# tho-kn/EgoTAP

Measured on AMD Instinct MI355X. Metric: stereo frames/sec (2D->3D lift, B=256, 256x256), higher is better.
Workload: dtype f32; 1 GPU; UnrealEgo 16-joint lifting head (heatmaps [B,90,64,64] -> joints [B,16,3]), forward only, fp32, batch 256 per GPU, inputs resident in HBM; batch_per_gpu=256, global_batch=256, heatmap=64, parallelism=dp1 (batch shards, no collective)

## Files before the change

### egotap_amd/csrc/egotap_abi.hip

```cpp
#include <stdarg.h>
#include <stdio.h>
#include <string.h>

#include <string>
#include <unordered_map>
#include <vector>

#include "attention_f32.h"
#include "common.h"
#include "conv_f32.h"
#include "conv_bf16.h"
#include "gemm_f32.h"
#include "gemm_bf16.h"
#include "gemm_bf16_dma.h"
#include "gemm_f32_dma.h"
#include "attention_bf16.h"
#include "layernorm.h"
#include "metrics.h"
#include "heatmap_synth.h"
#include "pu_chain.h"
#include "gemm_tn_bf16.h"
#include "train_ops.h"
#include "gemm_bf16s.h"
#include "gemm_bf16s64.h"
// ... 86 lines not shown

struct HmParams {
    struct Bn { const float *g, *b, *m, *v; long long* nbt; };
    const float* stem_w; Bn stem_bn;
    struct Block { const float *w1, *w2, *wd; Bn bn1, bn2, bnd; } blk[4][6];
    int nblk[4];
    struct Cv { const float *w, *b; } l1x1[4], up[3], head;
    int n_out;
};

struct egotap_handle_s {
    egotap_config cfg;
    int J, T, grid, ppd, side, seq, C, D, H, hid, out_joints;
    std::unordered_map<std::string, int64_t> expect[EGOTAP_NET_COUNT];
    std::unordered_map<std::string, Param> bound[EGOTAP_NET_COUNT];
    bool lift_resolved = false;
    LiftParams lp;
    std::unordered_map<std::string, Param> bound_grad;
    bool grad_resolved = false;
    LiftParams lg;
    bool hm_resolved[EGOTAP_NET_COUNT] = {false, false, false};
    HmParams hp[EGOTAP_NET_COUNT];
    int debug_stop = 0;
    int pu_resident[2] = {-1, -1};
    bool pu_chain = true;
    unsigned* pu_fault_host = nullptr;
    unsigned* pu_fault_dev = nullptr;
    int pu_faults = 0;
    int pu_debug_drop = 0;
    int precision = EGOTAP_PREC_F32;
    __bf16* wscratch = nullptr;
    size_t wscratch_bytes = 0;
    __bf16* ascratch = nullptr;
    size_t ascratch_bytes = 0;
    __bf16* conv_pack = nullptr;
    float* conv_part = nullptr;
    size_t conv_part_floats = 0;
    bool timing = false;
    std::vector<hipEvent_t> ev;
    struct Rec { const char* role; const char* kernel; double flops; };
    std::vector<Rec> rec;
    size_t ev_used = 0;
    std::string detail;
};
typedef egotap_handle_s Handle;

// ... 276 lines not shown
        : h(h_), s(s_), on(h_ && h_->timing) {
        if (!on) return;
        if (h->ev_used + 2 > h->ev.size()) {
            hipEvent_t a, b;
            if (hipEventCreate(&a) != hipSuccess || hipEventCreate(&b) != hipSuccess) { on = false; return; }
            h->ev.push_back(a);
            h->ev.push_back(b);
        }
        (void)hipEventRecord(h->ev[h->ev_used], s);
        h->rec.push_back({role, kernel, flops});
    }
    ~GemmTimer() {
        if (!on) return;
        (void)hipEventRecord(h->ev[h->ev_used + 1], s);
        h->ev_used += 2;
    }
};

template <class AL> struct AlName;
template <> struct AlName<ALoadPlain> { static constexpr const char* v = "ALoadPlain"; };
template <> struct AlName<ALoadPatch> { static constexpr const char* v = "ALoadPatch"; };
template <> struct AlName<ALoadTokens> { static constexpr const char* v = "ALoadTokens"; };
template <> struct AlName<ALoadLive> { static constexpr const char* v = "ALoadLive"; };
template <> struct AlName<ALoadRot> { static constexpr const char* v = "ALoadRot"; };
template <> struct AlName<ALoadStereo> { static constexpr const char* v = "ALoadStereo"; };
template <> struct AlName<ALoadStereoGated> { static constexpr const char* v = "ALoadStereoGated"; };
template <class E> struct EpiName;
template <> struct EpiName<EpiBias> { static constexpr const char* v = "EpiBias"; };
template <> struct EpiName<EpiBiasRes> { static constexpr const char* v = "EpiBiasRes"; };
template <> struct EpiName<EpiBiasResLive> { static constexpr const char* v = "EpiBiasResLive"; };
template <> struct EpiName<EpiBiasGelu> { static constexpr const char* v = "EpiBiasGelu"; };
template <> struct EpiName<EpiBnLrelu> { static constexpr const char* v = "EpiBnLrelu"; };
template <> struct EpiName<EpiPatch> { static constexpr const char* v = "EpiPatch"; };

template <class Cfg, class AL, class Epi>
static hipError_t gemm(Handle* h, const char* role, const AL& al, const SegMat& W, const Epi& epi, float* C, long ldc,
                       int M, int N, int K, hipStream_t s) {
    static const std::string kname = std::string("gemm_f32_kernel<") + std::to_string(Cfg::BM) + "x" +
                                     std::to_string(Cfg::BN) + "x" + std::to_string(Cfg::BK) + "," + AlName<AL>::v + "," +
                                     EpiName<Epi>::v + ">";
    GemmTimer t(h, s, role, kname.c_str(), 2.0 * M * N * K);
    return gemm_f32_launch<Cfg, AL, Epi>(al, W, epi, C, ldc, M, N, K, s);
}

static int device_cu_count() {
    static int n = 0;
    if (n == 0) {
        int dev = 0, v = 0;
        if (hipGetDevice(&dev) == hipSuccess && hipDeviceGetAttribute(&v, hipDeviceAttributeMultiprocessorCount, dev) == hipSuccess && v > 0) n = v;
        else n = 256;
    }
    return n;
}
// ... 36 lines not shown
        hipError_t e = hipGetLastError();
        if (e != hipSuccess) return e;
        if constexpr (std::is_same<AL, ALoadPlain>::value) {
            if (K % DmaCfg::BK == 0 && N % DmaCfg::BN == 0 && W.seg % DmaCfg::BN == 0 && al.lda % 4 == 0 && M >= 1024) {
                __bf16* a = (size_t)M * K * 2 <= h->ascratch_bytes ? h->ascratch : nullptr;
                if (a) {
                    const long a8 = (long)M * K / 8;
                    hipLaunchKernelGGL(f32_to_bf16_rows_kernel, dim3((unsigned)((a8 + 255) / 256)), dim3(256), 0, s, al.A, al.lda, a, K / 8, a8);
                    e = hipGetLastError();
                    if (e != hipSuccess) return e;
                    return gemm_bf16_dma_launch(a, (long)K, B, epi, C, ldc, M, N, K, device_cu_count(), s);
                }
            }
        }
        return gemm_bf16_persist_launch<BfCfg<1, 1>, AL, Epi, SegMatB>(al, B, epi, C, ldc, M, N, K, device_cu_count(), s);
    }
    return gemm_bf16_persist_launch<BfCfg<1, 1>, AL, Epi>(al, W, epi, C, ldc, M, N, K, device_cu_count(), s);
}

template <class AL, class Epi>
static hipError_t gemm_big(Handle* h, const char* role, const AL& al, const SegMat& W, const Epi& epi, float* C, long ldc,
                           int M, int N, int K, hipStream_t s) {
    using Cfg = PipeD;
    if (h && h->precision == EGOTAP_PREC_BF16X3) {
        static const std::string kname3 = std::string("gemm_bf16_persist_kernel<256x256x16,bf16x3,") + AlName<AL>::v + "," + EpiName<Epi>::v + ">";
        GemmTimer t(h, s, role, kname3.c_str(), 2.0 * M * N * K);
        return gemm_bf16_persist_launch<BfCfg<3, 1>, AL, Epi>(al, W, epi, C, ldc, M, N, K, device_cu_count(), s);
    }
    if (h && h->precision == EGOTAP_PREC_BF16) {
        static const std::string kname1 = std::string("gemm_bf16_persist_kernel<256x256x32,bf16,") + AlName<AL>::v + "," + EpiName<Epi>::v + ">";
        GemmTimer t(h, s, role, kname1.c_str(), 2.0 * M * N * K);
        return gemm_bf16_plain(h, al, W, epi, C, ldc, M, N, K, s);
    }
    if constexpr (AL::HAS_PTR) {
        if (N % DmaF32Cfg::BN == 0 && K % DmaF32Cfg::BK == 0 && W.seg % DmaF32Cfg::BN == 0 && W.ld % 4 == 0 && al.dma_ok()) {
            static const std::string kdma = std::string("gemm_f32_dma_kernel<256x256x16,") + AlName<AL>::v + "," + EpiName<Epi>::v + ">";
            GemmTimer t(h, s, role, kdma.c_str(), 2.0 * M * N * K);
            return gemm_f32_dma_launch(al, W, epi, C, ldc, M, N, K, device_cu_count(), s);
        }
    }
    static const std::string kname = std::string("gemm_f32_persist_kernel<256x256x16,") + AlName<AL>::v + "," + EpiName<Epi>::v + ">";
    GemmTimer t(h, s, role, kname.c_str(), 2.0 * M * N * K);
    return gemm_f32_persist_launch<Cfg, AL, Epi>(al, W, epi, C, ldc, M, N, K, device_cu_count(), s);
}

static constexpr size_t SPLITK_FLOATS = (size_t)1 << 24;
enum { GS_BIG = 0, GS_DIRECT_A, GS_DIRECT_S, GS_SPLIT_S, GS_SPLIT_A, GS_HYBRID };
struct SmallRoute { int kind, splits, head_rows; };
template <class E> struct epi_row_free : std::false_type {};
template <> struct epi_row_free<EpiBias> : std::true_type {};
template <> struct epi_row_free<EpiBiasGelu> : std::true_type {};
template <> struct epi_row_free<EpiBnLrelu> : std::true_type {};
template <> struct epi_row_free<EpiNone> : std::true_type {};
static SmallRoute gemm_small_route(const Handle* h, bool plain_loader, int M, int N, int K, int wseg, int cus, bool row_free = false) {
    const long tiles256 = (long)((M + 255) / 256) * ((N + 255) / 256);
    const long fill = (h && h->precision != EGOTAP_PREC_F32) ? 64 : 160;
    if (N % 128 != 0 || K % 32 != 0 || wseg % 128 != 0) return SmallRoute{GS_BIG, 1, 0};
    if (tiles256 >= fill) {
        if (plain_loader && h && h->precision == EGOTAP_PREC_F32 && tiles256 < 4L * cus) {
            const double t_round = K * 0.2319 + 5.0;
            const double t_big = (double)((tiles256 + cus - 1) / cus) * t_round;
            const double t_direct = gemm_f32_direct_estimate_us<TileA>(M, N, K, cus);
            if (row_free && N % 256 == 0 && tiles256 > cus) {
                const int tn = N / 256, mh = (int)((tiles256 / cus) * cus / tn);
                const int Mt = M - mh * 256;
                if (mh >= 1 && Mt > 0) {
// ... 102 lines not shown
    w.HPB = w.HPA + al256((size_t)B * H * 4);
    w.FAULT = take(64);
    w.SPLITK = take(SPLITK_FLOATS);
    w.total = o;
    return w;
}

#if EGOTAP_IN(0)
extern "C" int egotap_lift_workspace_bytes(egotap_handle h, int B, size_t* bytes) {
    EGO_CHECK(h && bytes, "null argument");
    EGO_CHECK(B >= 0, "negative batch");
    *bytes = lift_ws(h, B > 0 ? B : 1).total;
    return EGOTAP_OK;
}
#endif

#if EGOTAP_IN(0)
extern "C" int egotap_lift_intermediate(egotap_handle h, int B, const char* name, size_t* offset, int64_t* numel) {
    EGO_CHECK(h && name && offset && numel, "null argument");
    const LiftWs w = lift_ws(h, B > 0 ? B : 1);
    const int64_t M = (int64_t)B * h->seq;
    if (!strcmp(name, "tokens")) { *offset = w.Y; *numel = M * h->D; }
    else if (!strcmp(name, "x")) { *offset = w.X; *numel = M * h->D; }
    else if (!strcmp(name, "pos_embed")) { *offset = w.POSZ; *numel = (int64_t)B * h->T * h->hid; }
    else if (!strcmp(name, "rot_embed")) { *offset = w.ROTZ; *numel = (int64_t)B * h->T * h->hid; }
    else if (!strcmp(name, "skel_embed")) { *offset = w.HS1; *numel = (int64_t)h->J * B * h->H; }
    else { egotap_set_error("unknown intermediate '%s'", name); return EGOTAP_ERR_INVALID; }
    return EGOTAP_OK;
}
#endif

#if EGOTAP_IN(0)
extern "C" int egotap_set_pu_chain(egotap_handle h, int enable) {
    EGO_CHECK(h, "null handle");
    h->pu_chain = enable != 0;
    h->pu_resident[0] = h->pu_resident[1] = -1;
    return EGOTAP_OK;
}
extern "C" int egotap_debug_pu_drop_workgroups(egotap_handle h, int n) {
    EGO_CHECK(h && n >= 0 && n < 16, "egotap_debug_pu_drop_workgroups: n in [0, 16)");
    h->pu_debug_drop = n;
    return EGOTAP_OK;
}
extern "C" int egotap_pu_chain_status(egotap_handle h, int* enabled, int* faults) {
    EGO_CHECK(h, "null handle");
    if (h->pu_fault_host && __atomic_load_n(h->pu_fault_host, __ATOMIC_RELAXED) != 0u) {
// ... 18 lines not shown
extern "C" int egotap_set_weight_scratch(egotap_handle h, void* buf, size_t bytes) {
    EGO_CHECK(h, "null handle");
    EGO_CHECK(((uintptr_t)buf & 15) == 0, "egotap_set_weight_scratch: 16-byte alignment");
    h->wscratch = (__bf16*)buf;
    h->wscratch_bytes = buf ? bytes : 0;
    return EGOTAP_OK;
}
#endif

#if EGOTAP_IN(0)
extern "C" int egotap_set_act_scratch(egotap_handle h, void* buf, size_t bytes) {
    EGO_CHECK(h, "null handle");
    EGO_CHECK(((uintptr_t)buf & 15) == 0, "egotap_set_act_scratch: 16-byte alignment");
    h->ascratch = (__bf16*)buf;
    h->ascratch_bytes = buf ? bytes : 0;
    return EGOTAP_OK;
}
#endif

#if EGOTAP_IN(0)
extern "C" int egotap_lift_debug_stop(egotap_handle h, int stage) {
    EGO_CHECK(h, "null handle");
    h->debug_stop = stage;
    return EGOTAP_OK;
}
#endif

template <class Epi>
static hipError_t fc1_nt(Handle* h, int which, const __bf16* src, const __bf16* w, long K, const Epi& ep, int BT, int cus, hipStream_t s) {
    const int HW = h->cfg.hm_size * h->cfg.hm_size;
    const bool deep = g_gemm_bf16s_bk != 32 && K % 64 == 0 && K >= 128 && (which == 0 ? h->D % 64 == 0 : HW % 64 == 0) && (long)256 * K * 2 < (1L << 31);
    if (which == 0) {
        const size_t tok_bytes = (size_t)(BT / h->T) * h->seq * h->D * 2;
        if (deep && g_conv_addressing == 0 && tok_bytes < ((size_t)1 << 32) - 4096)
            return gemm_bf16s64_launch_x(X64TokensS{src, 0u, h->T, h->D, h->seq, h->side, h->ppd, h->grid}, w, K, ep, BT, 2048, (int)K, cus, s);
        if (deep) return gemm_bf16s64_launch_x(X64Tokens{src, h->T, h->D, h->seq, h->side, h->ppd, h->grid}, w, K, ep, BT, 2048, (int)K, cus, s);
        return gemm_bf16s_launch(XTokens{src, h->T, h->D, h->seq, h->side, h->ppd, h->grid}, w, K, ep, BT, 2048, (int)K, cus, s);
    }
    const size_t hm_bytes = (size_t)(BT / (2 * h->J)) * h->C * HW * 2;
    if (deep && g_conv_addressing == 0 && hm_bytes < ((size_t)1 << 32) - 4096) return gemm_bf16s64_launch_x(X64RotS{src, 0u, h->C, h->J, HW}, w, K, ep, BT, 2048, (int)K, cus, s);
    if (deep) return gemm_bf16s64_launch_x(X64Rot{src, h->C, h->J, HW}, w, K, ep, BT, 2048, (int)K, cus, s);
    return gemm_bf16s_launch(XRot{src, h->C, h->J, HW}, w, K, ep, BT, 2048, (int)K, cus, s);
}

static hipError_t launch_ln(const float* x, float* y, const float* g, const float* b, int rows, float eps, hipStream_t s) {
    if (rows <= 0) return hipSuccess;
// ... 9 lines not shown
        const SmallRoute r = gemm_small_route(h, true, M, D, K, D, device_cu_count());
        if ((r.kind == GS_SPLIT_S || r.kind == GS_SPLIT_A) && r.splits > 1) {
            static const std::string kname = "gemm_f32_splitk_kernel<ALoadPlain>+splitk_reduce_res_ln_kernel";
            GemmTimer t(h, s, role, kname.c_str(), 2.0 * M * D * K);
            hipError_t e = r.kind == GS_SPLIT_S ? gemm_f32_splitk_partials<TileS>(ALoadPlain{A, lda}, segmat1(Wp, D, K), P, SPLITK_FLOATS, M, D, K, s, r.splits)
                                                : gemm_f32_splitk_partials<TileA>(ALoadPlain{A, lda}, segmat1(Wp, D, K), P, SPLITK_FLOATS, M, D, K, s, r.splits);
            if (e != hipSuccess) return e;
            hipLaunchKernelGGL(splitk_reduce_res_ln_kernel<1024>, dim3(min((M + 3) / 4, 256 * 8)), dim3(256), 0, s, (const float*)P, bias, (const float*)X, X, ln_g,
                               ln_b, Y, M, r.splits, 1e-12f);
            return hipGetLastError();
        }
    }
    hipError_t e = gemm_small(h, role, ALoadPlain{A, lda}, segmat1(Wp, D, K), EpiBiasRes{segvec1(bias, D), X, D}, X, D, M, D, K, P, s);
    if (e != hipSuccess) return e;
    return launch_ln(X, Y, ln_g, ln_b, M, 1e-12f, s);
}

static ALoadPlain rebase(const ALoadPlain& a, int m0) { return ALoadPlain{a.A + (long)m0 * a.lda, a.lda}; }
static ALoadLive rebase(ALoadLive a, int m0) { a.lr.m0 += m0; return a; }
static EpiBias rebase(const EpiBias& e, int) { return e; }
static EpiBiasGelu rebase(const EpiBiasGelu& e, int) { return e; }
static EpiBiasRes rebase(EpiBiasRes e, int m0) { e.R += (long)m0 * e.ldr; return e; }
static EpiBiasResLive rebase(EpiBiasResLive e, int m0) { e.lr.m0 += m0; return e; }
template <class AL, class Epi>
static hipError_t gemm_rounds(Handle* h, const char* role, const AL& al, const SegMat& W, const Epi& epi, float* C, long ldc, int M, int N, int K,
                              hipStream_t s) {
    const int cus = device_cu_count(), tn = N / 256;
    const long tiles = (long)((M + 255) / 256) * tn;
    const int mh = (int)((tiles / cus) * cus / tn) * 256;
    if (N % 256 == 0 && K % 32 == 0 && mh > 0 && mh < M) {
        const double t_round = K * 0.2319 + 5.0;
        const double t_big = (double)((tiles + cus - 1) / cus) * t_round;
        const double t_split = (double)(((long)(mh / 256) * tn + cus - 1) / cus) * t_round + 4.0 + gemm_f32_direct_estimate_us<TileA>(M - mh, N, K, cus);
        if (t_split < t_big) {
            hipError_t e = gemm_big(h, role, al, W, epi, C, ldc, mh, N, K, s);
            if (e != hipSuccess) return e;
            return gemm<TileA>(h, role, rebase(al, mh), W, rebase(epi, mh), C + (long)mh * ldc, ldc, M - mh, N, K, s);
        }
    }
    return gemm_big(h, role, al, W, epi, C, ldc, M, N, K, s);
}

static bool lift_prune_last(Handle* h, int B) {
#ifdef EGOTAP_ATTN_F32_LIVE
    const int D = h->D, M = B * h->seq, Nq = h->T * h->ppd * h->ppd;
    if (h->precision != EGOTAP_PREC_F32 || h->debug_stop != 0 || h->cfg.vit_layers < 1 || Nq < 32 || Nq >= h->seq || D % 256 != 0) return false;
    const int cus = device_cu_count();
    if (gemm_small_route(h, true, M, 3 * D, D, D, cus, true).kind != GS_BIG || gemm_small_route(h, true, M, D, D, D, cus).kind != GS_BIG ||
        gemm_small_route(h, true, M, 4 * D, D, 4 * D, cus, true).kind != GS_BIG || gemm_small_route(h, true, M, D, 4 * D, D, cus).kind != GS_BIG)
        return false;
    return attention_f32_ksplit(B, h->seq, h->cfg.vit_heads, SPLITK_FLOATS, cus) == 1;
#else
    (void)h; (void)B;
    return false;
#endif
}

static int lift_forward_impl(Handle* h, const float* hm, int B, float* pose, void* ws, size_t ws_bytes, void* stream, bool pose_only,
                             const char* who) {
    EGO_CHECK(h, "null handle");
    if (B == 0) return EGOTAP_OK;
    EGO_CHECK(B > 0 && hm && pose && ws, "%s: null argument or negative batch", who);
    EGO_CHECK(((uintptr_t)hm & 15) == 0 && ((uintptr_t)ws & 255) == 0, "hm must be 16-byte and ws 256-byte aligned");
    int rc = lift_resolve(h);
    if (rc != EGOTAP_OK) return rc;
    const LiftWs w = lift_ws(h, B);
    if (ws_bytes < w.total) {
        egotap_set_error("workspace too small: %zu bytes given, %zu needed for B=%d", ws_bytes, w.total, B);
        return EGOTAP_ERR_WORKSPACE;
    }
    hipStream_t s = (hipStream_t)stream;
    const LiftParams& p = h->lp;
    char* base = (char*)ws;
    auto F = [&](size_t off) { return (float*)(base + off); };
    float *X = F(w.X), *Y = F(w.Y), *QKV = F(w.QKV), *CTX = F(w.CTX), *HID = F(w.HID);
    float* SPK = F(w.SPLITK);
    float *Z1 = F(w.Z1), *Z2 = F(w.Z2), *POSZ = F(w.POSZ), *ROTZ = F(w.ROTZ);
    float *F0 = F(w.F0), *G0 = F(w.G0), *HS0 = F(w.HS0), *F1 = F(w.F1), *G1 = F(w.G1), *HS1 = F(w.HS1);
// ... 63 lines not shown
            const XTokens xt{Yb, h->T, D, h->seq, h->side, h->ppd, h->grid};
            const int sp = gemm_bf16s_ksplit(BT, 2048, K1, cu, SPLITK_FLOATS);
            if (sp > 1) EGO_HIP(gemm_bf16s_splitk_launch(xt, Wb, (long)K1, bnf(p.pos_fc[0], Z1), SPK, sp, BT, 2048, K1, cu, s));
            else EGO_HIP(fc1_nt(h, 0, Yb, Wb, (long)K1, bnf(p.pos_fc[0], Z1), BT, cu, s));
            EGO_HIP((fc_gemm(h, "pos_fc2", ALoadPlain{Z1, 2048}, segmat1(p.pos_fc[1].w, 512, 2048), bn(p.pos_fc[1]), Z2, 512, BT, 512, 2048, SPK, s)));
            EGO_HIP((fc_gemm(h, "pos_fc3", ALoadPlain{Z2, 512}, segmat1(p.pos_fc[2].w, hid, 512), bn(p.pos_fc[2]), POSZ, hid, BT, hid, 512, SPK, s)));
        }
        {
            __bf16* hmb = HIDb;
            const long n8 = (long)B * h->C * HW / 8;
            hipLaunchKernelGGL(f32_to_bf16_kernel, dim3((unsigned)((n8 + 255) / 256)), dim3(256), 0, s, hm, hmb, n8);
            prep(p.rot_fc[0].w, Wb, 2048, 2 * HW);
            EGO_HIP(hipGetLastError());
            const XRot xr{hmb, h->C, J, HW};
            const int sp = gemm_bf16s_ksplit(BT, 2048, 2 * HW, cu, SPLITK_FLOATS);
            if (sp > 1) EGO_HIP(gemm_bf16s_splitk_launch(xr, Wb, 2L * HW, bnf(p.rot_fc[0], Z1), SPK, sp, BT, 2048, 2 * HW, cu, s));
            else EGO_HIP(fc1_nt(h, 1, hmb, Wb, 2L * HW, bnf(p.rot_fc[0], Z1), BT, cu, s));
            EGO_HIP((fc_gemm(h, "rot_fc2", ALoadPlain{Z1, 2048}, segmat1(p.rot_fc[1].w, 512, 2048), bn(p.rot_fc[1]), Z2, 512, BT, 512, 2048, SPK, s)));
            EGO_HIP((fc_gemm(h, "rot_fc3", ALoadPlain{Z2, 512}, segmat1(p.rot_fc[2].w, hid, 512), bn(p.rot_fc[2]), ROTZ, hid, BT, hid, 512, SPK, s)));
        }
    } else {
    const int NL = h->cfg.vit_layers;
    const bool prune = pose_only && lift_prune_last(h, B);
    EGO_HIP(launch_ln(X, Y, NL > 0 ? p.layer[0].ln1_g : p.lnf_g, NL > 0 ? p.layer[0].ln1_b : p.lnf_b, M, 1e-12f, s));
    for (int i = 0; i < NL; ++i) {
        const auto& L = p.layer[i];
#ifdef EGOTAP_ATTN_F32_LIVE
        if (prune && i + 1 == NL) {
            const LiveRows lr{h->seq, h->side, h->ppd, h->grid, h->T};
            const int Nq = h->T * h->ppd * h->ppd, Mc = B * Nq;
            float* Xc = QKV;
            SegMat Wkv; Wkv.p[0] = L.k_w; Wkv.p[1] = L.v_w; Wkv.p[2] = L.v_w; Wkv.seg = D; Wkv.ld = D;
            SegVec bkv; bkv.p[0] = L.k_b; bkv.p[1] = L.v_b; bkv.p[2] = L.v_b; bkv.seg = D;
            EGO_HIP((gemm_big(h, "kv", ALoadPlain{Y, D}, Wkv, EpiBias{bkv}, QKV + D, 3L * D, M, 2 * D, D, s)));
            EGO_HIP((gemm_rounds(h, "q_live", ALoadLive{Y, D, lr}, segmat1(L.q_w, D, D), EpiBias{segvec1(L.q_b, D)}, QKV, 3L * D, Mc, D, D, s)));
            EGO_HIP(attention_f32_live_launch(QKV, 3L * D, Nq, QKV, CTX, B, h->seq, h->cfg.vit_heads, s));
            EGO_HIP((gemm_rounds(h, "attn_out_live", ALoadPlain{CTX, D}, segmat1(L.o_w, D, D), EpiBiasResLive{segvec1(L.o_b, D), X, D, lr}, Xc, D, Mc, D, D, s)));
            EGO_HIP(launch_ln(Xc, Y, L.ln2_g, L.ln2_b, Mc, 1e-12f, s));
            EGO_HIP((gemm_rounds(h, "mlp_up_live", ALoadPlain{Y, D}, segmat1(L.up_w, 4 * D, D), EpiBiasGelu{segvec1(L.up_b, 4 * D)}, HID, 4L * D, Mc, 4 * D, D, s)));
            EGO_HIP((gemm_rounds(h, "mlp_down_live", ALoadPlain{HID, 4L * D}, segmat1(L.dn_w, D, 4 * D), EpiBiasRes{segvec1(L.dn_b, D), Xc, D}, Xc, D, Mc, D, 4 * D, s)));
            EGO_HIP(launch_ln(Xc, Y, p.lnf_g, p.lnf_b, Mc, 1e-12f, s));
            break;
        }
#endif
        {
            SegMat Wqkv; Wqkv.p[0] = L.q_w; Wqkv.p[1] = L.k_w; Wqkv.p[2] = L.v_w; Wqkv.seg = D; Wqkv.ld = D;
            SegVec bqkv; bqkv.p[0] = L.q_b; bqkv.p[1] = L.k_b; bqkv.p[2] = L.v_b; bqkv.seg = D;
            EGO_HIP((gemm_small(h, "qkv", ALoadPlain{Y, D}, Wqkv, EpiBias{bqkv}, QKV, 3L * D, M, 3 * D, D, SPK, s)));
        }
        if (h->precision == EGOTAP_PREC_BF16X3 && h->seq % 32 == 0) EGO_HIP(attention_bf16_launch<3>(QKV, CTX, B, h->seq, h->cfg.vit_heads, s));
        else if (h->precision == EGOTAP_PREC_BF16 && h->seq % 32 == 0) EGO_HIP(attention_bf16_launch<1>(QKV, CTX, B, h->seq, h->cfg.vit_heads, s));
        else EGO_HIP(attention_f32_launch(QKV, CTX, B, h->seq, h->cfg.vit_heads, s, nullptr, SPK, SPLITK_FLOATS, device_cu_count()));
        EGO_HIP(gemm_res_ln(h, "attn_out", CTX, D, L.o_w, L.o_b, X, M, D, D, L.ln2_g, L.ln2_b, Y, SPK, s));
        EGO_HIP((gemm_small(h, "mlp_up", ALoadPlain{Y, D}, segmat1(L.up_w, 4 * D, D), EpiBiasGelu{segvec1(L.up_b, 4 * D)}, HID, 4L * D, M, 4 * D, D, SPK, s)));
        const bool last = i + 1 == NL;
        EGO_HIP(gemm_res_ln(h, "mlp_down", HID, 4L * D, L.dn_w, L.dn_b, X, M, D, 4 * D, last ? p.lnf_g : p.layer[i + 1].ln1_g, last ? p.lnf_b : p.layer[i + 1].ln1_b, Y,
                            SPK, s));
        if (h->debug_stop == 2 + i) return EGOTAP_OK;
    }
    auto bn = [](const LiftParams::Fc& f) { return EpiBnLrelu{f.b, f.g, f.beta, f.mean, f.var, 1e-5f, 0.2f}; };
    const bool skinny_fc1 = BT < SKINNY_ROWS || (h->precision == EGOTAP_PREC_F32 && (long)((BT + 255) / 256) * (2048 / 256) < 100);
    {
        const int K1 = h->ppd * h->ppd * D;
        auto fc1 = [&](const auto& al) -> hipError_t {
            if (skinny_fc1 && BT <= 64)
                return gemm_f32_splitk_launch<TileS>(al, segmat1(p.pos_fc[0].w, 2048, K1), bn(p.pos_fc[0]), Z1, 2048, SPK, SPLITK_FLOATS, BT, 2048, K1, s, device_cu_count());
            if (skinny_fc1)
                return gemm_f32_splitk_launch<TileA>(al, segmat1(p.pos_fc[0].w, 2048, K1), bn(p.pos_fc[0]), Z1, 2048, SPK, SPLITK_FLOATS, BT, 2048, K1, s);
            return gemm_big(h, "pos_fc1", al, segmat1(p.pos_fc[0].w, 2048, K1), bn(p.pos_fc[0]), Z1, 2048, BT, 2048, K1, s);
        };
        if (prune) EGO_HIP(fc1(ALoadPlain{Y, (long)K1}));
// ... 2556 lines not shown
```

### egotap_amd/csrc/gemm_f32.h

```cpp
#pragma once
#include "common.h"
#include <type_traits>

struct ALoadPlain {
    const float* A;
    long lda;
    struct Row { const float* p; };
    __device__ __forceinline__ Row row(int m) const { return Row{A + (long)m * lda}; }
    __device__ __forceinline__ f32x4 load(const Row& r, int k) const { return *(const f32x4*)(r.p + k); }
    static constexpr bool HAS_PTR = true;
    __device__ __forceinline__ const float* ptr(const Row& r, int k) const { return r.p + k; }
    __host__ bool dma_ok() const { return lda % 4 == 0 && lda < (1L << 21) && ((uintptr_t)A & 15) == 0; }
};

struct ALoadPatch {
    const float* hm;
    int C, S, seq, side, ppd, grid, T;
    const float* zeros = nullptr;
    struct Row { const float* p; };
    static constexpr bool HAS_PTR = true;
    __device__ __forceinline__ const float* ptr(const Row& r, int k) const { return r.p ? r.p + (k >> 4) * S + (k & 15) : zeros + k; }
    __host__ bool dma_ok() const { return zeros != nullptr && S % 4 == 0 && ((uintptr_t)hm & 15) == 0 && ((uintptr_t)zeros & 15) == 0; }
    __device__ __forceinline__ Row row(int m) const {
        const int b = m / seq, tok = m - b * seq;
// ... 33 lines not shown
struct LiveRows {
    int seq, side, ppd, grid, T;
    int m0 = 0;
    __host__ __device__ __forceinline__ long phys(int m) const {
        m += m0;
        const int pp = ppd * ppd, L = T * pp;
        const int b = m / L, r = m - b * L, i = r / pp, s = r - i * pp;
        const int pr = (i / grid) * ppd + s / ppd, pc = (i % grid) * ppd + s % ppd;
        return (long)b * seq + pr * side + pc;
    }
};
struct ALoadLive {
    const float* A;
    long lda;
    LiveRows lr;
    struct Row { const float* p; };
    __device__ __forceinline__ Row row(int m) const { return Row{A + lr.phys(m) * lda}; }
    __device__ __forceinline__ f32x4 load(const Row& r, int k) const { return *(const f32x4*)(r.p + k); }
    static constexpr bool HAS_PTR = true;
    __device__ __forceinline__ const float* ptr(const Row& r, int k) const { return r.p + k; }
    __host__ bool dma_ok() const { return lda % 4 == 0 && lda < (1L << 21) && ((uintptr_t)A & 15) == 0; }
};

struct ALoadRot {
    const float* hm;
    int C, J, HW;
    struct Row { const float* p; };
    __device__ __forceinline__ Row row(int m) const {
        const int T = 2 * J;
        const int b = m / T, t = m - b * T;
        const int eye = t / J, j = t - eye * J;
        return Row{hm + (long)(b * C + 2 * J + eye * 2 * J + j) * HW};
    }
    __device__ __forceinline__ f32x4 load(const Row& r, int k) const {
        const int cs = k / HW;
        return *(const f32x4*)(r.p + (long)cs * J * HW + (k - cs * HW));
    }
    static constexpr bool HAS_PTR = true;
    __device__ __forceinline__ const float* ptr(const Row& r, int k) const {
        const int cs = k / HW;
        return r.p + (long)cs * J * HW + (k - cs * HW);
    }
    __host__ bool dma_ok() const { return HW % 4 == 0 && ((uintptr_t)hm & 15) == 0; }
};

struct ALoadStereo {
// ... 204 lines not shown
};

struct EpiScatterPatch : EpiNone {
    float* hm;
    int C, S, seq, side, ppd, grid, T;
    __device__ __forceinline__ float* dst(int m, int n) const {
        const int b = m / seq, tok = m - b * seq;
        const int pr = tok / side, pc = tok - pr * side;
        const int cell = (pr / ppd) * grid + pc / ppd;
        if (cell >= T) return nullptr;
        return hm + ((long)(b * C + cell) * S + (pr % ppd) * 16 + (n >> 4)) * S + (pc % ppd) * 16 + (n & 15);
    }
};
struct EpiScatterRot : EpiNone {
    float* hm;
    int C, J, HW;
    __device__ __forceinline__ float* dst(int m, int n) const {
        const int T = 2 * J;
        const int b = m / T, t = m - b * T;
        const int eye = t / J, j = t - eye * J, cs = n / HW;
        return hm + (long)(b * C + 2 * J + eye * 2 * J + cs * J + j) * HW + (n - cs * HW);
    }
};
template <class E> struct epi_scatters : std::false_type {};
template <> struct epi_scatters<EpiScatterPatch> : std::true_type {};
template <> struct epi_scatters<EpiScatterRot> : std::true_type {};
template <class Epi>
__device__ __forceinline__ void epi_store(const Epi& epi, float* C, long ldc, int m, int n, float v) {
    if constexpr (epi_scatters<Epi>::value) {
        if (float* p = epi.dst(m, n)) *p = v;
    } else {
        C[(long)m * ldc + n] = v;
    }
}
template <class Epi>
__device__ __forceinline__ void epi_store4(const Epi& epi, float* C, long ldc, int m, int n0, const f32x4& v) {
    if constexpr (epi_scatters<Epi>::value) {
        if (float* p = epi.dst(m, n0)) *(f32x4*)p = v;
    } else {
        *(f32x4*)(C + (long)m * ldc + n0) = v;
    }
}

template <int BM_, int BN_, int BK_, int WM_, int WN_, int MINW_>
struct GemmCfg {
    static constexpr int BM = BM_, BN = BN_, BK = BK_, WM = WM_, WN = WN_, MINW = MINW_;
    static constexpr int THREADS = 64 * WM * WN;
// ... 648 lines not shown
```

### egotap_amd/csrc/gemm_f32_dma.h

```cpp
#pragma once
#include <type_traits>
#include "gemm_f32.h"
#include "lds_dma.h"

struct DmaF32Cfg {
    static constexpr int BM = 256, BN = 256, BK = 16, WM = 4, WN = 2, THREADS = 512, NS = 4, TM = 2, TN = 4;
    static constexpr int ROWB = 64;
    static constexpr int STAGE = (BM + BN) * ROWB;
    static constexpr int ELD = 36, EPATCH = 16 * ELD * 4;
    static constexpr int LDS_BYTES = NS * STAGE + (THREADS / 64) * EPATCH;
    static_assert(LDS_BYTES <= 160 * 1024, "LDS budget");
};

template <class ALoad, class Epi>
__global__ __launch_bounds__(DmaF32Cfg::THREADS, 2) void gemm_f32_dma_kernel(ALoad al, SegMat W, Epi epi, float* C,
                                                                          long ldc, int M, int N, int K, int tiles_m, int tiles_n) {
    using Cfg = DmaF32Cfg;
    constexpr int BM = Cfg::BM, BN = Cfg::BN, BK = Cfg::BK, NS = Cfg::NS, TM = Cfg::TM, TN = Cfg::TN, ROWB = Cfg::ROWB, ELD = Cfg::ELD;
    extern __shared__ __attribute__((aligned(16))) char smem_dmaf[];
    const int tid = threadIdx.x, lane = tid & 63, wid = tid >> 6;
    const int wm = wid / Cfg::WN, wn = wid % Cfg::WN;
    const int l31 = lane & 31, lh = lane >> 5;
    float* Es = (float*)(smem_dmaf + NS * Cfg::STAGE + wid * Cfg::EPATCH);

// ... 194 lines not shown
            after_epi = true;
            {
                int tm_, tn_;
                tile_of(c_tile, tm_, tn_);
                constexpr bool DUAL = sizeof(typename Epi::Col4) <= 16 && !(Epi::HAS_RES && sizeof(typename Epi::Col4) < 16);
                if (DUAL && (tm_ + 1) * BM <= M) epilogue(std::integral_constant<bool, DUAL>{});
                else epilogue(std::false_type{});
            }
            c_kt = 0;
            ++c_tile;
        }
    }
    asm volatile("s_waitcnt vmcnt(0)" ::: "memory");
}

template <class ALoad, class Epi>
static hipError_t gemm_f32_dma_launch(const ALoad& al, const SegMat& W, const Epi& epi, float* C, long ldc, int M, int N, int K,
                                       int num_cu, hipStream_t stream) {
    using Cfg = DmaF32Cfg;
    if (M <= 0) return hipSuccess;
    if (N % Cfg::BN != 0 || K % Cfg::BK != 0 || W.seg % Cfg::BN != 0 || !al.dma_ok() || W.ld % 4 != 0) return hipErrorInvalidValue;
    if (W.ld >= (1L << 21) || K >= (1 << 21)) return hipErrorInvalidValue;
    auto kern = gemm_f32_dma_kernel<ALoad, Epi>;
    static bool attr_done = false;
    if (!attr_done) {
        hipError_t e = hipFuncSetAttribute((const void*)kern, hipFuncAttributeMaxDynamicSharedMemorySize, Cfg::LDS_BYTES);
        if (e != hipSuccess) return e;
        attr_done = true;
    }
    const int tiles_m = (M + Cfg::BM - 1) / Cfg::BM, tiles_n = N / Cfg::BN;
    const int ntiles = tiles_m * tiles_n;
    const int grid = ntiles < num_cu ? ntiles : num_cu;
    hipLaunchKernelGGL(kern, dim3(grid), dim3(Cfg::THREADS), Cfg::LDS_BYTES, stream, al, W, epi, C, ldc, M, N, K, tiles_m, tiles_n);
    return hipGetLastError();
}
```

### egotap_amd/lib.py

```python
from __future__ import annotations

import ctypes as C
import os

from . import build as _build

ERR_NAMES = {1: "EGOTAP_ERR_INVALID", 2: "EGOTAP_ERR_HIP", 3: "EGOTAP_ERR_UNBOUND", 4: "EGOTAP_ERR_WORKSPACE"}
NET_LIFT, NET_HM_POS, NET_HM_ROT = 0, 1, 2
F32, I64 = 0, 1
PRECISIONS = {"f32": 0, "bf16x3": 1, "bf16": 2}


class EgotapConfig(C.Structure):
    _fields_ = [(n, C.c_int32) for n in (
        "struct_bytes", "n_joints_hm", "estimate_head", "hm_size", "hidden", "vit_dim", "vit_heads", "vit_layers",
        "patch", "pu_hidden")] + [("hm_blocks", C.c_int32 * 4)]


class EgotapError(RuntimeError):
    pass


_lib = None

_PROTOS = {
    "egotap_abi_version": (C.c_int, []),
    "egotap_last_error": (C.c_char_p, []),
    "egotap_create": (C.c_int, [C.POINTER(EgotapConfig), C.POINTER(C.c_void_p)]),
    "egotap_destroy": (None, [C.c_void_p]),
    "egotap_bind_param": (C.c_int, [C.c_void_p, C.c_int, C.c_char_p, C.c_void_p, C.c_int64, C.c_int]),
    "egotap_unbound_count": (C.c_int, [C.c_void_p, C.c_int, C.POINTER(C.c_int)]),
    "egotap_lift_workspace_bytes": (C.c_int, [C.c_void_p, C.c_int, C.POINTER(C.c_size_t)]),
    "egotap_lift_forward": (C.c_int, [C.c_void_p, C.c_void_p, C.c_int, C.c_void_p, C.c_void_p, C.c_size_t, C.c_void_p]),
    "egotap_lift_predict_pose": (C.c_int, [C.c_void_p, C.c_void_p, C.c_int, C.c_void_p, C.c_void_p, C.c_size_t, C.c_void_p]),
    "egotap_lift_intermediate": (C.c_int, [C.c_void_p, C.c_int, C.c_char_p, C.POINTER(C.c_size_t), C.POINTER(C.c_int64)]),
    "egotap_lift_debug_stop": (C.c_int, [C.c_void_p, C.c_int]),
    "egotap_set_precision": (C.c_int, [C.c_void_p, C.c_int]),
    "egotap_set_pu_chain": (C.c_int, [C.c_void_p, C.c_int]),
    "egotap_pu_chain_status": (C.c_int, [C.c_void_p, C.POINTER(C.c_int), C.POINTER(C.c_int)]),
    "egotap_debug_pu_drop_workgroups": (C.c_int, [C.c_void_p, C.c_int]),
    "egotap_debug_gemm_bk": (C.c_int, [C.c_int]),
    "egotap_debug_conv_addressing": (C.c_int, [C.c_int]),
    "egotap_set_weight_scratch": (C.c_int, [C.c_void_p, C.c_void_p, C.c_size_t]),
    "egotap_set_act_scratch": (C.c_int, [C.c_void_p, C.c_void_p, C.c_size_t]),
    "egotap_hm_workspace_bytes": (C.c_int, [C.c_void_p, C.c_int, C.POINTER(C.c_size_t)]),
    "egotap_hm_forward": (C.c_int, [C.c_void_p, C.c_int, C.c_void_p, C.c_void_p, C.c_int, C.c_void_p, C.c_int64, C.c_void_p,
                                    C.c_size_t, C.c_void_p]),
    "egotap_hm_intermediate": (C.c_int, [C.c_void_p, C.c_int, C.c_char_p, C.POINTER(C.c_size_t), C.POINTER(C.c_int64)]),
    "egotap_hm_forward_bnbatch_workspace_bytes": (C.c_int, [C.c_void_p, C.c_int, C.c_int, C.POINTER(C.c_size_t)]),
    "egotap_hm_forward_bnbatch_intermediate": (C.c_int, [C.c_void_p, C.c_int, C.c_int, C.c_char_p, C.POINTER(C.c_size_t), C.POINTER(C.c_int64)]),
    "egotap_hm_forward_bnbatch": (C.c_int, [C.c_void_p, C.c_int, C.c_void_p, C.c_void_p, C.c_int, C.c_void_p, C.c_int64, C.c_int, C.c_void_p,
                                            C.c_size_t, C.c_void_p]),
    "egotap_linear_f32": (C.c_int, [C.c_void_p] * 4 + [C.c_int] * 4 + [C.c_void_p] * 5 + [C.c_int, C.c_void_p]),
    "egotap_gemm_tile_name": (C.c_char_p, [C.c_int]),
    "egotap_linear_bf16_dma": (C.c_int, [C.c_void_p] * 4 + [C.c_int] * 3 + [C.c_void_p]),
    "egotap_layernorm_f32": (C.c_int, [C.c_void_p] * 4 + [C.c_int, C.c_int, C.c_float, C.c_void_p]),
    "egotap_attention_f32": (C.c_int, [C.c_void_p, C.c_void_p, C.c_int, C.c_int, C.c_int, C.c_void_p]),
    "egotap_pose_metrics": (C.c_int, [C.c_void_p, C.c_void_p, C.c_int, C.c_int, C.c_void_p, C.c_void_p, C.c_void_p, C.c_void_p]),
    "egotap_pose_metrics_batch_axes": (C.c_int, [C.c_void_p, C.c_void_p, C.c_int, C.c_int, C.c_void_p, C.c_void_p, C.c_void_p, C.c_void_p]),
# ... 221 lines not shown
```

### include/egotap_debug.h

```cpp
#ifndef EGOTAP_DEBUG_H
#define EGOTAP_DEBUG_H
#include "egotap.h"

#ifdef __cplusplus
extern "C" {
#endif

int egotap_debug_pu_drop_workgroups(egotap_handle h, int n);

int egotap_lift_debug_stop(egotap_handle h, int stage);

int egotap_debug_gemm_bk(int bk);

int egotap_debug_conv_addressing(int mode);

int egotap_debug_wgrad_splits(int tiles, int64_t slabs, int64_t n_floats, size_t slab_bytes, int num_cu, int lds_bytes, double slab_us, double fixed_us,
                              int* per);

int egotap_timing_enable(egotap_handle h, int enable);
int egotap_timing_read(egotap_handle h, int* launches, double* total_ms, double* total_flops);
const char* egotap_timing_detail(egotap_handle h);

#ifdef __cplusplus
}
#endif
#endif
```

Baseline: 2886 stereo frames/s.

## Compute layer-0 QKV for batch-invariant rows once and broadcast

```diff
diff --git a/egotap_amd/csrc/egotap_abi.hip b/egotap_amd/csrc/egotap_abi.hip
--- a/egotap_amd/csrc/egotap_abi.hip
+++ b/egotap_amd/csrc/egotap_abi.hip
@@ -132,6 +132,7 @@
     bool hm_resolved[EGOTAP_NET_COUNT] = {false, false, false};
     HmParams hp[EGOTAP_NET_COUNT];
     int debug_stop = 0;
+    bool share_layer0 = true;
     int pu_resident[2] = {-1, -1};
     bool pu_chain = true;
     unsigned* pu_fault_host = nullptr;
@@ -454,6 +455,7 @@
 template <> struct AlName<ALoadPatch> { static constexpr const char* v = "ALoadPatch"; };
 template <> struct AlName<ALoadTokens> { static constexpr const char* v = "ALoadTokens"; };
 template <> struct AlName<ALoadLive> { static constexpr const char* v = "ALoadLive"; };
+template <> struct AlName<ALoadLayer0> { static constexpr const char* v = "ALoadLayer0"; };
 template <> struct AlName<ALoadRot> { static constexpr const char* v = "ALoadRot"; };
 template <> struct AlName<ALoadStereo> { static constexpr const char* v = "ALoadStereo"; };
 template <> struct AlName<ALoadStereoGated> { static constexpr const char* v = "ALoadStereoGated"; };
@@ -461,6 +463,7 @@
 template <> struct EpiName<EpiBias> { static constexpr const char* v = "EpiBias"; };
 template <> struct EpiName<EpiBiasRes> { static constexpr const char* v = "EpiBiasRes"; };
 template <> struct EpiName<EpiBiasResLive> { static constexpr const char* v = "EpiBiasResLive"; };
+template <> struct EpiName<EpiBiasLayer0> { static constexpr const char* v = "EpiBiasLayer0"; };
 template <> struct EpiName<EpiBiasGelu> { static constexpr const char* v = "EpiBiasGelu"; };
 template <> struct EpiName<EpiBnLrelu> { static constexpr const char* v = "EpiBnLrelu"; };
 template <> struct EpiName<EpiPatch> { static constexpr const char* v = "EpiPatch"; };
@@ -543,6 +546,14 @@
 static hipError_t gemm_big(Handle* h, const char* role, const AL& al, const SegMat& W, const Epi& epi, float* C, long ldc,
                            int M, int N, int K, hipStream_t s) {
     using Cfg = PipeD;
+    if constexpr (epi_scatters<Epi>::value) {
+        static_assert(AL::HAS_PTR, "scattering epilogues run on the LDS-DMA kernel");
+        if ((h && h->precision != EGOTAP_PREC_F32) || N % DmaF32Cfg::BN != 0 || K % DmaF32Cfg::BK != 0 || W.seg % DmaF32Cfg::BN != 0 || W.ld % 4 != 0 || !al.dma_ok())
+            return hipErrorInvalidValue;
+        static const std::string kdma = std::string("gemm_f32_dma_kernel<256x256x16,") + AlName<AL>::v + "," + EpiName<Epi>::v + ">";
+        GemmTimer t(h, s, role, kdma.c_str(), 2.0 * M * N * K);
+        return gemm_f32_dma_launch(al, W, epi, C, ldc, M, N, K, device_cu_count(), s);
+    } else {
     if (h && h->precision == EGOTAP_PREC_BF16X3) {
         static const std::string kname3 = std::string("gemm_bf16_persist_kernel<256x256x16,bf16x3,") + AlName<AL>::v + "," + EpiName<Epi>::v + ">";
         GemmTimer t(h, s, role, kname3.c_str(), 2.0 * M * N * K);
@@ -563,6 +574,7 @@
     static const std::string kname = std::string("gemm_f32_persist_kernel<256x256x16,") + AlName<AL>::v + "," + EpiName<Epi>::v + ">";
     GemmTimer t(h, s, role, kname.c_str(), 2.0 * M * N * K);
     return gemm_f32_persist_launch<Cfg, AL, Epi>(al, W, epi, C, ldc, M, N, K, device_cu_count(), s);
+    }
 }
 
 static constexpr size_t SPLITK_FLOATS = (size_t)1 << 24;
@@ -711,6 +723,7 @@
     const int64_t M = (int64_t)B * h->seq;
     if (!strcmp(name, "tokens")) { *offset = w.Y; *numel = M * h->D; }
     else if (!strcmp(name, "x")) { *offset = w.X; *numel = M * h->D; }
+    else if (!strcmp(name, "qkv")) { *offset = w.QKV; *numel = M * 3 * h->D; }
     else if (!strcmp(name, "pos_embed")) { *offset = w.POSZ; *numel = (int64_t)B * h->T * h->hid; }
     else if (!strcmp(name, "rot_embed")) { *offset = w.ROTZ; *numel = (int64_t)B * h->T * h->hid; }
     else if (!strcmp(name, "skel_embed")) { *offset = w.HS1; *numel = (int64_t)h->J * B * h->H; }
@@ -775,6 +788,11 @@
 extern "C" int egotap_lift_debug_stop(egotap_handle h, int stage) {
     EGO_CHECK(h, "null handle");
     h->debug_stop = stage;
+    return EGOTAP_OK;
+}
+extern "C" int egotap_lift_debug_share_layer0(egotap_handle h, int enable) {
+    EGO_CHECK(h, "null handle");
+    h->share_layer0 = enable != 0;
     return EGOTAP_OK;
 }
 #endif
@@ -830,6 +848,8 @@
 static EpiBiasGelu rebase(const EpiBiasGelu& e, int) { return e; }
 static EpiBiasRes rebase(EpiBiasRes e, int m0) { e.R += (long)m0 * e.ldr; return e; }
 static EpiBiasResLive rebase(EpiBiasResLive e, int m0) { e.lr.m0 += m0; return e; }
+static ALoadLayer0 rebase(ALoadLayer0 a, int m0) { a.lr.m0 += m0; return a; }
+static EpiBiasLayer0 rebase(EpiBiasLayer0 e, int m0) { e.lr.m0 += m0; return e; }
 template <class AL, class Epi>
 static hipError_t gemm_rounds(Handle* h, const char* role, const AL& al, const SegMat& W, const Epi& epi, float* C, long ldc, int M, int N, int K,
                               hipStream_t s) {
@@ -862,6 +882,23 @@
     (void)h; (void)B;
     return false;
 #endif
+}
+
+static bool lift_share_layer0(Handle* h, int B) {
+    const int D = h->D, Nq = h->T * h->ppd * h->ppd;
+    if (!h->share_layer0 || h->precision != EGOTAP_PREC_F32 || h->cfg.vit_layers < 1 || Nq < 32 || Nq >= h->seq || D % 256 != 0 || B < 2) return false;
+    const int cus = device_cu_count();
+    if (gemm_small_route(h, true, B * h->seq, 3 * D, D, D, cus, true).kind != GS_BIG) return false;
+    const long tn = 3 * D / 256, full = (long)((B * h->seq + 255) / 256) * tn, live = (long)((B * Nq + h->seq - Nq + 255) / 256) * tn;
+    return (live + cus - 1) / cus < (full + cus - 1) / cus;
+}
+static __global__ __launch_bounds__(256) void lift_bcast_rows_kernel(float* __restrict__ C, int n4, Layer0Rows lr, int B) {
+    const long row = lr.phys(lr.Mc + blockIdx.x);
+    const f32x4* src = (const f32x4*)(C + row * 4L * n4);
+    for (int c = threadIdx.x; c < n4; c += 256) {
+        const f32x4 v = src[c];
+        for (int b = 1 + blockIdx.y; b < B; b += gridDim.y) ((f32x4*)(C + ((long)b * lr.seq + row) * 4L * n4))[c] = v;
+    }
 }
 
 static int lift_forward_impl(Handle* h, const float* hm, int B, float* pose, void* ws, size_t ws_bytes, void* stream, bool pose_only,
@@ -971,6 +1008,7 @@
     } else {
     const int NL = h->cfg.vit_layers;
     const bool prune = pose_only && lift_prune_last(h, B);
+    const bool share0 = lift_share_layer0(h, B);
     EGO_HIP(launch_ln(X, Y, NL > 0 ? p.layer[0].ln1_g : p.lnf_g, NL > 0 ? p.layer[0].ln1_b : p.lnf_b, M, 1e-12f, s));
     for (int i = 0; i < NL; ++i) {
         const auto& L = p.layer[i];
@@ -995,7 +1033,22 @@
         {
             SegMat Wqkv; Wqkv.p[0] = L.q_w; Wqkv.p[1] = L.k_w; Wqkv.p[2] = L.v_w; Wqkv.seg = D; Wqkv.ld = D;
             SegVec bqkv; bqkv.p[0] = L.q_b; bqkv.p[1] = L.k_b; bqkv.p[2] = L.v_b; bqkv.seg = D;
-            EGO_HIP((gemm_small(h, "qkv", ALoadPlain{Y, D}, Wqkv, EpiBias{bqkv}, QKV, 3L * D, M, 3 * D, D, SPK, s)));
+            if (i == 0 && share0) {
+                const int Nq = h->T * h->ppd * h->ppd, Mc = B * Nq, Nd = h->seq - Nq;
+                const Layer0Rows lr{h->seq, h->side, h->ppd, h->grid, h->T, Mc};
+                {
+                    GemmTimer t(h, s, "qkv", "gemm_f32_dma_kernel<256x256x16,ALoadLayer0,EpiBiasLayer0>", 2.0 * (Mc + Nd) * 3 * D * D);
+                    const bool timing = h->timing;
+                    h->timing = false;
+                    const hipError_t e = gemm_rounds(h, "qkv", ALoadLayer0{Y, D, lr}, Wqkv, EpiBiasLayer0{{bqkv}, QKV, 3L * D, lr}, QKV, 3L * D, Mc + Nd, 3 * D, D, s);
+                    h->timing = timing;
+                    EGO_HIP(e);
+                }
+                hipLaunchKernelGGL(lift_bcast_rows_kernel, dim3(Nd, min(B - 1, 16)), dim3(256), 0, s, QKV, 3 * D / 4, lr, B);
+                EGO_HIP(hipGetLastError());
+            } else {
+                EGO_HIP((gemm_small(h, "qkv", ALoadPlain{Y, D}, Wqkv, EpiBias{bqkv}, QKV, 3L * D, M, 3 * D, D, SPK, s)));
+            }
         }
         if (h->precision == EGOTAP_PREC_BF16X3 && h->seq % 32 == 0) EGO_HIP(attention_bf16_launch<3>(QKV, CTX, B, h->seq, h->cfg.vit_heads, s));
         else if (h->precision == EGOTAP_PREC_BF16 && h->seq % 32 == 0) EGO_HIP(attention_bf16_launch<1>(QKV, CTX, B, h->seq, h->cfg.vit_heads, s));
diff --git a/egotap_amd/csrc/gemm_f32.h b/egotap_amd/csrc/gemm_f32.h
--- a/egotap_amd/csrc/gemm_f32.h
+++ b/egotap_amd/csrc/gemm_f32.h
@@ -79,6 +79,31 @@
     __host__ bool dma_ok() const { return lda % 4 == 0 && lda < (1L << 21) && ((uintptr_t)A & 15) == 0; }
 };
 
+struct Layer0Rows {
+    int seq, side, ppd, grid, T, Mc;
+    int m0 = 0;
+    __host__ __device__ __forceinline__ long phys(int m) const {
+        m += m0;
+        const int pp = ppd * ppd, L = T * pp;
+        int b = 0, r = L + (m - Mc);
+        if (m < Mc) { b = m / L; r = m - b * L; }
+        const int i = r / pp, s = r - i * pp;
+        const int pr = (i / grid) * ppd + s / ppd, pc = (i % grid) * ppd + s % ppd;
+        return (long)b * seq + pr * side + pc;
+    }
+};
+struct ALoadLayer0 {
+    const float* A;
+    long lda;
+    Layer0Rows lr;
+    struct Row { const float* p; };
+    __device__ __forceinline__ Row row(int m) const { return Row{A + lr.phys(m) * lda}; }
+    __device__ __forceinline__ f32x4 load(const Row& r, int k) const { return *(const f32x4*)(r.p + k); }
+    static constexpr bool HAS_PTR = true;
+    __device__ __forceinline__ const float* ptr(const Row& r, int k) const { return r.p + k; }
+    __host__ bool dma_ok() const { return lda % 4 == 0 && lda < (1L << 21) && ((uintptr_t)A & 15) == 0; }
+};
+
 struct ALoadRot {
     const float* hm;
     int C, J, HW;
@@ -329,7 +354,14 @@
         return hm + (long)(b * C + 2 * J + eye * 2 * J + cs * J + j) * HW + (n - cs * HW);
     }
 };
+struct EpiBiasLayer0 : EpiBias {
+    float* Cp;
+    long ldcp;
+    Layer0Rows lr;
+    __device__ __forceinline__ float* dst(int m, int n) const { return Cp + lr.phys(m) * ldcp + n; }
+};
 template <class E> struct epi_scatters : std::false_type {};
+template <> struct epi_scatters<EpiBiasLayer0> : std::true_type {};
 template <> struct epi_scatters<EpiScatterPatch> : std::true_type {};
 template <> struct epi_scatters<EpiScatterRot> : std::true_type {};
 template <class Epi>
diff --git a/egotap_amd/csrc/gemm_f32_dma.h b/egotap_amd/csrc/gemm_f32_dma.h
--- a/egotap_amd/csrc/gemm_f32_dma.h
+++ b/egotap_amd/csrc/gemm_f32_dma.h
@@ -240,11 +240,13 @@
     if (N % Cfg::BN != 0 || K % Cfg::BK != 0 || W.seg % Cfg::BN != 0 || !al.dma_ok() || W.ld % 4 != 0) return hipErrorInvalidValue;
     if (W.ld >= (1L << 21) || K >= (1 << 21)) return hipErrorInvalidValue;
     auto kern = gemm_f32_dma_kernel<ALoad, Epi>;
-    static bool attr_done = false;
-    if (!attr_done) {
+    static bool attr_done[64] = {};
+    int dev = 0;
+    if (hipGetDevice(&dev) != hipSuccess || dev < 0) return hipErrorInvalidDevice;
+    if (dev >= 64 || !attr_done[dev]) {
         hipError_t e = hipFuncSetAttribute((const void*)kern, hipFuncAttributeMaxDynamicSharedMemorySize, Cfg::LDS_BYTES);
         if (e != hipSuccess) return e;
-        attr_done = true;
+        if (dev < 64) attr_done[dev] = true;
     }
     const int tiles_m = (M + Cfg::BM - 1) / Cfg::BM, tiles_n = N / Cfg::BN;
     const int ntiles = tiles_m * tiles_n;
diff --git a/egotap_amd/lib.py b/egotap_amd/lib.py
--- a/egotap_amd/lib.py
+++ b/egotap_amd/lib.py
@@ -35,6 +35,7 @@
     "egotap_lift_predict_pose": (C.c_int, [C.c_void_p, C.c_void_p, C.c_int, C.c_void_p, C.c_void_p, C.c_size_t, C.c_void_p]),
     "egotap_lift_intermediate": (C.c_int, [C.c_void_p, C.c_int, C.c_char_p, C.POINTER(C.c_size_t), C.POINTER(C.c_int64)]),
     "egotap_lift_debug_stop": (C.c_int, [C.c_void_p, C.c_int]),
+    "egotap_lift_debug_share_layer0": (C.c_int, [C.c_void_p, C.c_int]),
     "egotap_set_precision": (C.c_int, [C.c_void_p, C.c_int]),
     "egotap_set_pu_chain": (C.c_int, [C.c_void_p, C.c_int]),
     "egotap_pu_chain_status": (C.c_int, [C.c_void_p, C.POINTER(C.c_int), C.POINTER(C.c_int)]),
diff --git a/include/egotap_debug.h b/include/egotap_debug.h
--- a/include/egotap_debug.h
+++ b/include/egotap_debug.h
@@ -9,6 +9,7 @@
 int egotap_debug_pu_drop_workgroups(egotap_handle h, int n);
 
 int egotap_lift_debug_stop(egotap_handle h, int stage);
+int egotap_lift_debug_share_layer0(egotap_handle h, int enable);
 
 int egotap_debug_gemm_bk(int bk);
 
```

Result: no change. 2899 stereo frames/s, median of 6 (+0.5%).
